# georgeyounes/CRIMP

Measured on AMD Instinct MI355X. Metric: Z^2_2 photon*trial evals/sec (node), higher is better.
Workload: dtype f64; 1 GPU; config3: synthetic 10000000 photons x 1000000 trials/GPU, Z^2_2; photons=10000000, trials_per_gpu=1000000, nharm=2, parallelism=trial-sharded dp1: sharding.sharded_search + all_gather(best), precision=default

## Files before the change

### crimp_amd/csrc/search_nufft.h

```cpp
#pragma once

#include "search_nufft_plan.h"
#include "search_nufft_finish.h"

typedef double nu_f64x4 __attribute__((ext_vector_type(4)));

constexpr int kNuTile = 4096;
constexpr double kNuRho = 1e-13;

struct NuTw {
    const double2* lo;
    const double2* hi;
    int lbits;
    int64_t mask;
};

__device__ __forceinline__ double2 nu_cmul(double2 a, double2 b) {
    return make_double2(a.x * b.x - a.y * b.y, a.x * b.y + a.y * b.x);
}
__device__ __forceinline__ double2 nu_add(double2 a, double2 b) { return make_double2(a.x + b.x, a.y + b.y); }
__device__ __forceinline__ double2 nu_sub(double2 a, double2 b) { return make_double2(a.x - b.x, a.y - b.y); }
__device__ __forceinline__ double2 nu_muli(double2 a) { return make_double2(-a.y, a.x); }

__device__ __forceinline__ double2 nu_tw(const NuTw& T, int64_t t) {
// ... 730 lines not shown
        }
    }
    __syncthreads();
}

__device__ __forceinline__ void nu_fft_lds(double2* s, int ll, int lc, int sa, int sc, const NuTile* tw, int lt) {
    int lns = 0;
    while (lns < ll) {
        const int rem = ll - lns;
        if (rem >= 4) {
            nu_stage<16>(s, ll, lc, sa, sc, lns, tw, lt);
            lns += 4;
        } else if (rem == 3) {
            nu_stage<8>(s, ll, lc, sa, sc, lns, tw, lt);
            lns += 3;
        } else if (rem == 2) {
            nu_stage<4>(s, ll, lc, sa, sc, lns, tw, lt);
            lns += 2;
        } else {
            nu_stage<2>(s, ll, lc, sa, sc, lns, tw, lt);
            lns += 1;
        }
    }
}

__global__ __launch_bounds__(256) __attribute__((amdgpu_waves_per_eu(2))) void k_nu_fft_cols(const double2* __restrict__ X, double2* __restrict__ Y,
                                                     int lnfft, int ln1, int lc, NuTw T, int alo, int acnt) {
    extern __shared__ double2 nu_s[];
    __shared__ NuTile tw;
    const int lt = lnfft < 12 ? lnfft : 12;
    nu_tile_init(&tw, lt);
    const int ln2 = lnfft - ln1, c = 1 << lc, n1 = 1 << ln1;
    const int64_t nfft = int64_t(1) << lnfft;
    const int64_t b0 = (int64_t)blockIdx.x << lc;
    const double2* x = X + (int64_t)blockIdx.y * nfft;
    double2* y = Y + (int64_t)blockIdx.y * nfft;
    for (int e = threadIdx.x; e < (n1 << lc); e += 256) {
        const int a = e >> lc, cc = e & (c - 1);
        nu_s[e] = ((a - alo) & (n1 - 1)) < acnt ? x[((int64_t)a << ln2) + b0 + cc] : make_double2(0.0, 0.0);
    }
    __syncthreads();
    nu_fft_lds(nu_s, ln1, lc, c, 1, &tw, lt);
#pragma unroll
    for (int q = 0; q < kNuTile / 256; ++q) {
        const int e = threadIdx.x + 256 * q;
        if (e < (n1 << lc)) {
            const int k1 = e >> lc, cc = e & (c - 1);
            const int64_t b = b0 + cc;
            y[((int64_t)k1 << ln2) + b] = nu_cmul(nu_s[e], nu_tw(T, b * k1));
        }
    }
}

__global__ __launch_bounds__(256) __attribute__((amdgpu_waves_per_eu(2))) void k_nu_cols256(
    const double2* __restrict__ X, double2* __restrict__ Y, int lnfft, NuTw T, int alo, int acnt, int64_t ngroups) {
    extern __shared__ double2 nu_s[];
    __shared__ NuTile tw;
    nu_tile_init(&tw, 12);
    const int ln2 = lnfft - 8;
    const int64_t nfft = int64_t(1) << lnfft;
    const int cc = threadIdx.x & 15, j = threadIdx.x >> 4;
    const int64_t cpb = int64_t(1) << (ln2 - 4);
    double2 nv[16], tf[4];
    auto fetch = [&](int64_t grp) {
        const int64_t b = ((grp % cpb) << 4) + cc;
        const double2* x = X + (grp / cpb) * nfft + b;
        const int64_t lm = (int64_t(1) << T.lbits) - 1, tb = (b * (int64_t)j) & T.mask, ts = (b << 4) & T.mask;
        tf[0] = T.hi[tb >> T.lbits];
        tf[1] = T.lo[tb & lm];
        tf[2] = T.hi[ts >> T.lbits];
        tf[3] = T.lo[ts & lm];
#pragma unroll
        for (int r = 0; r < 16; ++r) {
            const int a = j + 16 * r;
            nv[r] = ((a - alo) & 255) < acnt ? x[(int64_t)a << ln2] : make_double2(0.0, 0.0);
        }
    };
    int64_t grp = blockIdx.x;
    if (grp < ngroups) fetch(grp);
    __syncthreads();
    for (; grp < ngroups; grp += gridDim.x) {
        double2 v[16];
#pragma unroll
        for (int r = 0; r < 16; ++r) v[r] = nv[r];
        const double2 wb = nu_cmul(tf[0], tf[1]), ws = nu_cmul(tf[2], tf[3]);
        const int64_t b = ((grp % cpb) << 4) + cc;
        double2* y = Y + (grp / cpb) * nfft + b;
        if (grp + gridDim.x < ngroups) fetch(grp + gridDim.x);
        nu_dft16(v);
#pragma unroll
        for (int r = 0; r < 16; ++r) nu_s[((j << 4) + r) * 16 + cc] = v[r];
        __syncthreads();
#pragma unroll
        for (int r = 0; r < 16; ++r) v[r] = nu_s[(j + 16 * r) * 16 + cc];
        __syncthreads();
        nu_twiddle<16>(nu_tw_tile(&tw, j << 4), v);
        nu_dft16(v);
        v[0] = nu_cmul(v[0], wb);
        nu_twiddle<16>(ws, v);
#pragma unroll
        for (int r = 1; r < 16; ++r) v[r] = nu_cmul(v[r], wb);
#pragma unroll
        for (int r = 0; r < 16; ++r) y[(int64_t)(j + 16 * r) << ln2] = v[r];
    }
}

__global__ __launch_bounds__(512) __attribute__((amdgpu_waves_per_eu(4))) void k_nu_cols512(
    const double2* __restrict__ X, double2* __restrict__ Y, int lnfft, NuTw T, int alo, int acnt, int64_t ngroups) {
    constexpr int NC = 1, C = 8;
    extern __shared__ double2 nu_s[];
    __shared__ NuTile tw;
    nu_tile_init(&tw, 9);
    const int ln2 = lnfft - 9;
    const int64_t nfft = int64_t(1) << lnfft;
    const int cc = threadIdx.x & 7, j = threadIdx.x >> 3;
    const int64_t cpb = int64_t(1) << (ln2 - 3);
    double2 nv[NC][8], tf[NC][4];
    const int voff = ((j << ln2) + cc) * 16;
    auto fetch = [&](int64_t grp) {
        const int64_t b0 = (grp % cpb) * C;
        const __amdgpu_buffer_rsrc_t rs = __builtin_amdgcn_make_buffer_rsrc(
            (void*)(X + (grp / cpb) * nfft + b0), (short)0, (int)(16 << lnfft), 0x00020000);
        const int64_t lm = (int64_t(1) << T.lbits) - 1;
#pragma unroll
        for (int c = 0; c < NC; ++c) {
            const int64_t b = b0 + cc + 8 * c, tb = (b * (int64_t)j) & T.mask, ts = (b << 6) & T.mask;
            tf[c][0] = T.hi[tb >> T.lbits];
            tf[c][1] = T.lo[tb & lm];
            tf[c][2] = T.hi[ts >> T.lbits];
            tf[c][3] = T.lo[ts & lm];
        }
#pragma unroll
        for (int q = 0; q < 8; ++q) {
            const bool occ = ((j + 64 * q - alo) & 511) < acnt;
#pragma unroll
            for (int c = 0; c < NC; ++c)
                nv[c][q] = occ ? __builtin_bit_cast(double2, __builtin_amdgcn_raw_buffer_load_b128(
                                                                 rs, voff, ((64 * q << ln2) + 8 * c) * 16, 0))
                               : make_double2(0.0, 0.0);
        }
    };
    int64_t grp = blockIdx.x;
    if (grp < ngroups) fetch(grp);
    const int m2 = (j & 7) << 3;
    const int z2 = ((j >> 3) << 6) + (j & 7);
    __syncthreads();
    typedef unsigned int nu_u4 __attribute__((ext_vector_type(4)));
    for (; grp < ngroups; grp += gridDim.x) {
        double2 v[NC][8], wb[NC], ws[NC];
#pragma unroll
        for (int c = 0; c < NC; ++c) {
#pragma unroll
            for (int q = 0; q < 8; ++q) v[c][q] = nv[c][q];
            wb[c] = nu_cmul(tf[c][0], tf[c][1]);
            ws[c] = nu_cmul(tf[c][2], tf[c][3]);
        }
// ... 78 lines not shown
    }
    for (int p = P - 1; p >= 0; --p) {
        const int64_t pn = (int64_t)(p > 0 ? p - 1 : 0) * pstride;
#pragma unroll
        for (int q = 0; q < kNuFusedPer; ++q) {
            const int e = threadIdx.x + 256 * q;
            if (e < L) {
                nu_s[e] = nx[q];
                nx[q] = xr[pn + e];
            }
        }
        __syncthreads();
        nu_fft_lds(nu_s, ll, 0, 1, L, &tw, lt);
#pragma unroll
        for (int q = 0; q < kNuFusedPer; ++q) {
            const int b = threadIdx.x + 256 * q;
            if (b < L) {
                const double2 v = nu_s[b];
                const int64_t J = k1 + ((int64_t)b << ln1);
                const int64_t jc = J <= jhi ? J : J - nfft;
                acc[q] = nu_bes_acc(acc[q], nu_bes_w(bs[q], p, nu_zh(jc, lnfft)), v, p);
            }
        }
        __syncthreads();
    }
#pragma unroll
    for (int q = 0; q < kNuFusedPer; ++q) {
        const int b = threadIdx.x + 256 * q;
        if (b >= L) continue;
        const int64_t J = k1 + ((int64_t)b << ln1);
        int64_t jc;
        if (J <= jhi)
            jc = J;
        else if (J >= nfft - h)
            jc = J - nfft;
        else
            continue;
        const int64_t t = tbase + r * nf + jc;
        if (t >= 0 && t < nbt) CS[t] = acc[q];
    }
}

struct NuFinal {
    int on, m, stat, Pc;
    double nph, invfact, rel;
    int64_t tb0;
    double* out;
    int* nflag;
    int64_t* flagged;
    BestCand* best_part;
    int64_t best_base;
    const double2* CS0;
};
template <int TPB, int NP>
__device__ __forceinline__ void nu_rows_epilogue(const double2 (&acc)[NP], int64_t k1, int ln1, int64_t nfft,
                                                 int64_t jhi, int64_t h, int64_t tbase, int r, int64_t nf, int64_t nbt,
                                                 double2* __restrict__ CS, const NuFinal& F, double2* lds,
                                                 int pos0 = -1) {
    const int t = threadIdx.x;
    const int b0 = pos0 < 0 ? t : pos0;
    if (!F.on) {
#pragma unroll
        for (int q = 0; q < NP; ++q) {
            const int64_t J = k1 + ((int64_t)(b0 + TPB * q) << ln1);
            int64_t jc;
            if (J <= jhi)
                jc = J;
            else if (J >= nfft - h)
                jc = J - nfft;
            else
                continue;
            const int64_t tt = tbase + r * nf + jc;
            if (tt >= 0 && tt < nbt) CS[tt] = acc[q];
        }
        return;
    }
    BestCand bc_ = {-INFINITY, INT64_MAX};
#pragma unroll
    for (int q = 0; q < NP; ++q) {
        const int64_t J = k1 + ((int64_t)(b0 + TPB * q) << ln1);
        int64_t jc;
        if (J <= jhi)
            jc = J;
        else if (J >= nfft - h)
            jc = J - nfft;
        else
            continue;
        const int64_t tt = tbase + r * nf + jc;
        if (tt < 0 || tt >= nbt) continue;
        double p, err;
        nu_power(F.CS0, nbt, tt, F.m, F.stat, F.nph, nu_err_bound(jc, nfft, F.Pc, F.invfact, F.nph), true, acc[q], &p,
                 &err);
        F.out[F.tb0 + tt] = p;
        if (!(err <= F.rel * fabs(p))) F.flagged[atomicAdd(F.nflag, 1)] = F.tb0 + tt;
        if (best_better(p, F.tb0 + tt, bc_.v, bc_.i)) bc_ = {p, F.tb0 + tt};
    }
    if (!F.best_part) return;
    for (int o = 32; o > 0; o >>= 1) {
        const double v = __shfl_xor(bc_.v, o);
        const int64_t i = __shfl_xor(bc_.i, o);
        if (best_better(v, i, bc_.v, bc_.i)) bc_ = {v, i};
    }
    __syncthreads();
    BestCand* red = reinterpret_cast<BestCand*>(lds);
    if ((t & 63) == 0) red[t >> 6] = bc_;
    __syncthreads();
    if (t == 0) {
        for (int w = 1; w < TPB / 64; ++w)
            if (best_better(red[w].v, red[w].i, bc_.v, bc_.i)) bc_ = red[w];
        F.best_part[F.best_base + (int64_t)blockIdx.y * gridDim.x + blockIdx.x] = bc_;
    }
}

struct NuRot {
// ... 61 lines not shown
        for (int q = 0; q < 8; ++q) v[q] = A[rd + TPB * 9 / 8 * q];
        nu_twiddle<8>(nu_tw_tile(&tw, m2), v);
        nu_dft8(v);
#pragma unroll
        for (int q = 0; q < 8; ++q) B[w2 + Ns2 * q + (q >> 1)] = v[q];
        __syncthreads();
#pragma unroll
        for (int q = 0; q < 8; ++q) v[q] = B[rd + TPB * 9 / 8 * q];
        nu_twiddle<8>(nu_tw_tile(&tw, m3), v);
        nu_dft8(v);
#pragma unroll
        for (int q = 0; q < 8; ++q) A[w3 + Ns3 * 9 / 8 * q] = v[q];
        __syncthreads();
#pragma unroll
        for (int q = 0; q < 8; ++q) v[q] = A[rd + TPB * 9 / 8 * q];
        nu_twiddle<8>(nu_tw_tile(&tw, m4), v);
        nu_dft8(v);
        const double pp1 = (double)(p + 1);
#pragma unroll
        for (int q = 0; q < 8; ++q) {
            const double j = fma(pp1 * bs[q].iz2, bs[q].j1, -bs[q].j2);
            bs[q].j2 = bs[q].j1;
            bs[q].j1 = j;
            double w = j;
            if constexpr (last) w = (q == 0 && k1 == 0 && t == 0) ? 1.0 : 0.5 * j;
            acc[q] = make_double2(fma(w, v[q].x, -acc[q].y), fma(w, v[q].y, acc[q].x));
        }
    };
    const int pend = plo > 0 ? plo : 1;
    int p = P - 1;
    double2* TA = nu_s;
    double2* TB = nu_s + NT;
    if (p >= pend && ((p - pend + 1) & 1)) {
        moment(std::false_type(), p, xa, xb, TA, TB);
        --p;
#pragma unroll
        for (int q = 0; q < 8; ++q) xa[q] = xb[q];
        double2* tt = TA;
        TA = TB;
        TB = tt;
    }
    for (; p >= pend; p -= 2) {
        moment(std::false_type(), p, xa, xb, TA, TB);
        moment(std::false_type(), p - 1, xb, xa, TB, TA);
    }
    if (plo == 0) moment(std::true_type(), 0, xa, xb, TA, TB);
    const int rl = plo & 3;
#pragma unroll
    for (int q = 0; q < 8; ++q) {
        const double2 a = acc[q];
        acc[q] = rl == 0 ? a : rl == 1 ? make_double2(-a.y, a.x) : rl == 2 ? make_double2(-a.x, -a.y)
                                                                : make_double2(a.y, -a.x);
    }
    nu_rows_epilogue<TPB, 8>(acc, k1, ln1, nfft, jhi, h, tbase, r, nf, nbt, CS, F, nu_s);
}

__global__ __launch_bounds__(512) __attribute__((amdgpu_waves_per_eu(2))) void k_nu_rows_iw(
    const double2* X, int lnfft, int P, int plo, int accum, int nrow, int64_t nf, int64_t jhi, int64_t h,
    int64_t tbase, int64_t nbt, const double* __restrict__ bc, double2* __restrict__ CS, const NuFinal F, int xcd) {
    constexpr int N = 4096, TPB = 512;
    extern __shared__ double2 nu_s[];
    __shared__ NuTile tw;
    nu_tile_init(&tw, 12);
    const int64_t nfft = int64_t(1) << lnfft;
    const int ln1 = lnfft - 12;
    const int64_t k1b = nu_row_of_block(blockIdx.x, 1u << ln1, xcd);
    const int r = blockIdx.y;
    const int t = threadIdx.x, w = t >> 6, L = t & 63, hi3 = L >> 3, lo3 = L & 7;
    const int pos0 = w + 8 * hi3 + 64 * lo3;
    const double2* xr = X + (int64_t)r * nfft + (k1b << 12);
    const int64_t pstride = (int64_t)nrow * nfft;
    auto load_row = [&](int pm, double2 (&dst)[8]) {
        const __amdgpu_buffer_rsrc_t rs =
            __builtin_amdgcn_make_buffer_rsrc((void*)(xr + (int64_t)pm * pstride), (short)0, N * 16, 0x00020000);
#pragma unroll
        for (int q = 0; q < 8; ++q)
            dst[q] = __builtin_bit_cast(double2, __builtin_amdgcn_raw_buffer_load_b128(rs, t * 16, TPB * 16 * q, 0));
    };
    double2 acc[8], xa[8], xb[8];
    NuRot bs[8];
    const int rP = P & 3;
#pragma unroll
    for (int q = 0; q < 8; ++q) {
        double2 a0 = make_double2(0.0, 0.0);
        const int64_t J = k1b + ((int64_t)(pos0 + TPB * q) << ln1);
        const int64_t jc = J <= jhi ? J : J - nfft;
        if (accum) {
            const int64_t tt = tbase + r * nf + jc;
            if ((J <= jhi || J >= nfft - h) && tt >= 0 && tt < nbt) a0 = CS[tt];
        }
        acc[q] = rP == 0 ? a0 : rP == 1 ? make_double2(a0.y, -a0.x) : rP == 2 ? make_double2(-a0.x, -a0.y)
                                                                        : make_double2(-a0.y, a0.x);
        const NuBes b0 = nu_bes_start(bc, P, nu_zh(jc, lnfft));
        bs[q] = {2.0 * b0.j1, 2.0 * b0.j2, b0.iz2};
    }
    load_row(P - 1 - plo, xa);
    const int cw = 64 * w + L, cr = 512 * w + L, e1w = 512 * w + 64 * hi3 + lo3, e2w = 512 * w + 8 * hi3,
              e2r = 512 * w + 64 * lo3 + 8 * hi3;
    __syncthreads();
    auto moment = [&](auto LAST, int p, double2 (&v)[8], double2 (&nv)[8], double2* A) {
        constexpr bool last = decltype(LAST)::value;
        if (p > plo) load_row(p - 1 - plo, nv);
        nu_dft8(v);
        nu_twiddle<8>(nu_tw_tile(&tw, t), v);
#pragma unroll
        for (int q = 0; q < 8; ++q) A[cw + 512 * q] = v[q];
        __syncthreads();
#pragma unroll
        for (int q = 0; q < 8; ++q) v[q] = A[cr + 64 * q];
        nu_dft8(v);
        nu_twiddle<8>(nu_tw_tile(&tw, 8 * L), v);
#pragma unroll
        for (int q = 0; q < 8; ++q) A[e1w + 8 * q] = v[q];
        asm volatile("s_waitcnt lgkmcnt(0)" ::: "memory");
#pragma unroll
        for (int q = 0; q < 8; ++q) v[q] = A[cr + 64 * q];
        nu_dft8(v);
        nu_twiddle<8>(nu_tw_tile(&tw, 64 * lo3), v);
#pragma unroll
        for (int q = 0; q < 8; ++q) A[e2w + 64 * q + (lo3 ^ q)] = v[q];
        asm volatile("s_waitcnt lgkmcnt(0)" ::: "memory");
#pragma unroll
        for (int q = 0; q < 8; ++q) v[q] = A[e2r + (q ^ lo3)];
        nu_dft8(v);
        const double pp1 = (double)(p + 1);
#pragma unroll
        for (int q = 0; q < 8; ++q) {
            const double j = fma(pp1 * bs[q].iz2, bs[q].j1, -bs[q].j2);
            bs[q].j2 = bs[q].j1;
            bs[q].j1 = j;
            double wgt = j;
            if constexpr (last) wgt = (q == 0 && k1b == 0 && pos0 == 0) ? 1.0 : 0.5 * j;
            acc[q] = make_double2(fma(wgt, v[q].x, -acc[q].y), fma(wgt, v[q].y, acc[q].x));
        }
    };
    const int pend = plo > 0 ? plo : 1;
    int p = P - 1;
    double2* TA = nu_s;
    double2* TB = nu_s + N;
    if (p >= pend && ((p - pend + 1) & 1)) {
        moment(std::false_type(), p, xa, xb, TA);
        --p;
#pragma unroll
        for (int q = 0; q < 8; ++q) xa[q] = xb[q];
        double2* tt = TA;
        TA = TB;
        TB = tt;
    }
    for (; p >= pend; p -= 2) {
        moment(std::false_type(), p, xa, xb, TA);
        moment(std::false_type(), p - 1, xb, xa, TB);
    }
    if (plo == 0) moment(std::true_type(), 0, xa, xb, TA);
    const int rl = plo & 3;
#pragma unroll
    for (int q = 0; q < 8; ++q) {
        const double2 a = acc[q];
        acc[q] = rl == 0 ? a : rl == 1 ? make_double2(-a.y, a.x) : rl == 2 ? make_double2(-a.x, -a.y)
                                                                : make_double2(a.y, -a.x);
    }
    nu_rows_epilogue<TPB, 8>(acc, k1b, ln1, nfft, jhi, h, tbase, r, nf, nbt, CS, F, nu_s, pos0);
}

__global__ __launch_bounds__(256) void k_nu_finalize(const double2* __restrict__ CS, int64_t nbt, int m, int stat,
                                                     double nph, int64_t nf, int64_t jbase, int64_t nfft, int P,
                                                     double invfact, double rel, int64_t tb0, int64_t first,
                                                     double* __restrict__ out, int* __restrict__ nflag,
                                                     int64_t* __restrict__ flagged) {
    const int64_t t = (int64_t)blockIdx.x * blockDim.x + threadIdx.x;
    if (t >= nbt) return;
    const int64_t flat = tb0 + t + first;
    const int64_t jc = flat % nf - jbase;
    double p, err;
    nu_power(CS, nbt, t, m, stat, nph, nu_err_bound(jc, nfft, P, invfact, nph), false, make_double2(0.0, 0.0), &p,
             &err);
    out[tb0 + t] = p;
    if (!(err <= rel * fabs(p))) flagged[atomicAdd(nflag, 1)] = tb0 + t;
}

static int g_last_search_path = 0;
static int64_t g_last_nufft_n = 0;
static int g_last_nufft_p = 0;
static int g_last_nufft_gather = 0;
static double g_nu_work[kNuCls] = {0, 0, 0, 0, 0, 0, 0};
static int64_t g_last_cells_built = 0, g_last_cells_reused = 0;

struct NuTables {
    NuTw T{};
    const double2* cis = nullptr;
    const double2* cis2 = nullptr;
    const double* bc = nullptr;
};
static int nu_tables(hipStream_t s, int lnfft, NuTables* out) {
    static std::mutex mu;
    static std::map<std::pair<int, int>, double2*> cache;
    const int lbits = std::min(lnfft, 11);
    const int64_t nlo = int64_t(1) << lbits, nhi = int64_t(1) << (lnfft - lbits);
    int dev = 0;
    HIPCHK(hipGetDevice(&dev));
    double2* d = nullptr;
    {
        std::lock_guard<std::mutex> lk(mu);
        auto it = cache.find({dev, lnfft});
        if (it != cache.end()) {
            d = it->second;
        } else {
            std::vector<double2> h((size_t)(nlo + nhi + 1024 + kNuBesP * kNuBesM / 2 + 2048));
            const long double tp = 6.283185307179586476925286766559L;
            const long double nf = (long double)(int64_t(1) << lnfft);
            for (int64_t i = 0; i < nlo; ++i) {
                const long double a = tp * (long double)i / nf;
                h[(size_t)i] = make_double2((double)cosl(a), (double)sinl(a));
            }
            for (int64_t i = 0; i < nhi; ++i) {
// ... 311 lines not shown
        else if (sp.starts_max > 0)
            HIPCHK(sc.alloc(&cstart, (size_t)sp.starts_max));
        HIPCHK(sc.alloc(&W, (size_t)(sp.Bmax * sp.gw)));
        HIPCHK(sc.alloc(&Y, (size_t)sp.Bmax));
        HIPCHK(sc.alloc(&CS, (size_t)sp.csmax));
        HIPCHK(sc.alloc(&flagged, (size_t)in.shape.count));
        if (best_host)
            best_part = reinterpret_cast<BestCand*>(reinterpret_cast<char*>(in.nflag) + kNuFinCandOff);
        else if (sp.best_alloc > 0)
            HIPCHK(sc.alloc(&best_part, (size_t)sp.best_alloc));
        if (!sp.passes.empty()) {
            HIPCHK(sc.alloc(&dps, sp.passes.size()));
            HIPCHK(hipMemcpyAsync(dps, sp.passes.data(), sp.passes.size() * sizeof(NuPass), hipMemcpyHostToDevice, s));
        }
        return CRIMP_OK;
    }

    int cell_starts(const NuGroup& g, int64_t base) {
        const int64_t n = in.shape.n;
        for (const NuCellLaunch& cl : g.cells) {
            NuCellArgs ca = cl.args;
            for (int j = 0; j < cl.nk; ++j) ca.off[j] += base;
            const unsigned cb = (unsigned)std::min<int64_t>(cdiv(cdiv(n, 2), 256 * kNuCellU), 2048);
            if ((reinterpret_cast<uintptr_t>(in.t) & 15u) == 0)
                k_nu_cellstart<true><<<cb, 256, 0, s>>>(in.t, in.t0, n, g.pl.s1, cl.k0, cl.nk, ca, cstart, in.nflag + 1);
            else
                k_nu_cellstart<false><<<cb, 256, 0, s>>>(in.t, in.t0, n, g.pl.s1, cl.k0, cl.nk, ca, cstart, in.nflag + 1);
            HIPCHK(hipGetLastError());
        }
        HIPCHK(span(kNuClsCellStart));
        return CRIMP_OK;
    }

    int gather_set(const NuGroup& g, const NuBatch& b, const NuGatherSet& set, int64_t base) {
        const NuPlan& pl = g.pl;
        NuGatherSet S = set;
        for (int jj = 0; jj < S.nk; ++jj) S.soff[jj] += base;
        NuFold F;
        if (fold) {
            char* blkp = reinterpret_cast<char*>(in.nflag);
            F.epoch = epoch;
            F.ncheck = first_gather ? ncheck : 0;
            F.f = in.freq;
            F.nf = in.shape.nf;
            F.n = in.shape.n;
            F.pub = reinterpret_cast<double*>(blkp + kNuFinPubOff);
            F.part = reinterpret_cast<double2*>(blkp + kNuFinPartOff);
        }
        first_gather = false;
        launch_gather(in.twod, cells_reuse, S.blk0[S.nk], in.t, in.t0, cstart, int64_t(1) << pl.lnfft, pl.s1, pl.fch,
                      pl.fcl, in.twod ? in.c2 + b.rb : nullptr, b.nrow, pl.P, S, in.nflag + 1, tab.cis2, W, F, s);
        HIPCHK(hipGetLastError());
        HIPCHK(span(kNuClsSpread));
        for (int jj = 0; jj < S.nk; ++jj) {
            const int rc = fft_combine(g, b, S.k[jj], W + S.woff[jj]);
            if (rc) return rc;
        }
        return CRIMP_OK;
    }

    int mfma_pass(const NuGroup& g, const NuBatch& b, const NuMfmaPass& mp) {
        const NuPlan& pl = g.pl;
        const int64_t n = in.shape.n, nchunk = sp.nchunk, nfft = int64_t(1) << pl.lnfft;
        const int64_t SL = 2 * (int64_t)pl.P * b.nrow;
        const NuPass& ps = sp.passes[mp.ipass];
        const NuPass* dp = dps + mp.ipass;
        const dim3 grid((unsigned)cdiv(nchunk, kNuWaves));
        if (in.twod)
            nu_launch_spread<true>(mp.gl, grid, s, in.t, in.t0, n, nchunk, pl.s1, pl.fch, pl.fcl, in.c2 + b.rb, b.nrow,
                                   mp.k0, pl.P, dp, tab.cis, U, ctab, in.nflag + 1);
        else
            nu_launch_spread<false>(mp.gl, grid, s, in.t, in.t0, n, nchunk, pl.s1, pl.fch, pl.fcl, in.c2 + b.rb, b.nrow,
                                    mp.k0, pl.P, dp, tab.cis, U, ctab, in.nflag + 1);
        HIPCHK(hipGetLastError());
        HIPCHK(span(kNuClsSpread));
        for (int kk = 0; kk < mp.gl && mp.k0 + kk <= in.shape.nharm; ++kk) {
            const int k = mp.k0 + kk;
            int alo = 0, acnt = 0;
            nu_occupied(pl.gmin[(size_t)(k - 1)], pl.gmax[(size_t)(k - 1)], pl.lnfft, g.ln1, &alo, &acnt);
            const int64_t gbase = (int64_t)alo << g.ln2, gcount = (int64_t)acnt << g.ln2;
            k_nu_merge<<<(unsigned)cdiv(gcount, kNuMergeG), 256, (size_t)kNuMergeG * SL * sizeof(double), s>>>(
                U + ps.ubase[kk], SL, ctab + 2 * kk * nchunk, nchunk, ps.gmin[kk], pl.gmax[(size_t)(k - 1)], nfft, gbase,
                gcount, W, in.nflag + 1);
            HIPCHK(hipGetLastError());
            HIPCHK(span(kNuClsMerge));
            const int rc = fft_combine(g, b, k, W);
            if (rc) return rc;
        }
        return CRIMP_OK;
    }

    int fft_combine(const NuGroup& g, const NuBatch& b, int k, const double2* Wk) {
        const NuPlan& pl = g.pl;
        const NuSearchShape& sh = in.shape;
        const bool generic_fft = in.hooks.generic_fft;
        const int lnfft = pl.lnfft, P = pl.P, ln1 = g.ln1, ln2 = g.ln2;
        const size_t lds_fft = (size_t)kNuTile * sizeof(double2);
        const int64_t Bp = (int64_t)P * b.nrow;
        const double2* Z = Wk;
        if (ln1 > 0) {
            const int lcol = 12 - ln1;
            int alo = 0, acnt = 0;
            nu_occupied(pl.gmin[(size_t)(k - 1)], pl.gmax[(size_t)(k - 1)], lnfft, ln1, &alo, &acnt);
            if (ln1 == 8 && !generic_fft) {
                const int64_t ngroups = Bp << (ln2 - 4);
                k_nu_cols256<<<(unsigned)std::min<int64_t>(ngroups, 2 * nu_cus()), 256, lds_fft, s>>>(
                    Wk, Y, lnfft, tab.T, alo, acnt, ngroups);
            } else if (ln1 == 9 && !generic_fft) {
                const int64_t ngroups = Bp << (ln2 - 3);
                k_nu_cols512<<<(unsigned)std::min<int64_t>(ngroups, 2 * nu_cus()), 512, lds_fft, s>>>(
                    Wk, Y, lnfft, tab.T, alo, acnt, ngroups);
            } else {
                k_nu_fft_cols<<<dim3((unsigned)(int64_t(1) << (ln2 - lcol)), (unsigned)Bp), 256, lds_fft, s>>>(
                    Wk, Y, lnfft, ln1, lcol, tab.T, alo, acnt);
            }
            HIPCHK(hipGetLastError());
            Z = Y;
            HIPCHK(span(kNuClsPass1));
        }
        NuFinal F{};
        if (g.fuse_final && k == sh.nharm) {
            F.on = 1;
            F.m = sh.nharm;
            F.stat = sh.stat;
            F.Pc = P;
            F.nph = (double)sh.n;
            F.invfact = pl.invfact;
            F.rel = in.search_hooks.fixup_rel;
            F.tb0 = b.tb0;
            F.out = in.out;
            F.nflag = in.nflag;
            F.flagged = flagged;
            F.best_part = in.best ? best_part : nullptr;
            F.best_base = b.best_base;
            F.CS0 = CS;
        }
        const dim3 g2((unsigned)(int64_t(1) << ln1), (unsigned)b.nrow);
        const int xcd = in.hooks.row_map;
        const int64_t jhi = pl.nseg - 1 - pl.h, tbase = b.rb * sh.nf + g.jbase - (b.tb0 + sh.first);
        double2* CSk = CS + (int64_t)(k - 1) * b.nbt;
        if (ln2 == 12 && !generic_fft)
            k_nu_rows_iw<<<g2, 512, 2 * lds_fft, s>>>(Z, lnfft, P, 0, 0, b.nrow, sh.nf, jhi, pl.h, tbase, b.nbt, tab.bc,
                                                      CSk, F, xcd);
        else if (ln2 == 11 && !generic_fft)
            k_nu_rows_combine8<11><<<g2, 256, nu_rows_lds(11), s>>>(Z, lnfft, P, 0, 0, b.nrow, sh.nf, jhi, pl.h, tbase,
                                                                     b.nbt, tab.bc, CSk, F);
        else
            k_nu_fft_rows_combine<<<g2, 256, lds_fft, s>>>(Z, ln2, lnfft, P, b.nrow, sh.nf, jhi, pl.h, tbase, b.nbt,
                                                           tab.bc, CSk, xcd);
        HIPCHK(hipGetLastError());
        HIPCHK(span(kNuClsPass2));
        return CRIMP_OK;
    }

    int finalize(const NuGroup& g, const NuBatch& b) {
        const NuSearchShape& sh = in.shape;
        k_nu_finalize<<<(unsigned)cdiv(b.nbt, 256), 256, 0, s>>>(CS, b.nbt, sh.nharm, sh.stat, (double)sh.n, sh.nf, g.jbase,
                                                                 int64_t(1) << g.pl.lnfft, g.pl.P, g.pl.invfact,
                                                                 in.search_hooks.fixup_rel, b.tb0, sh.first, in.out, in.nflag, flagged);
        HIPCHK(hipGetLastError());
        HIPCHK(span(kNuClsFinalize));
        return CRIMP_OK;
    }

    int launch_all() {
        int cur_lnfft = -1;
        for (const NuGroup& g : sp.groups) {
            int rc = CRIMP_OK;
            if (g.pl.lnfft != cur_lnfft) {
                rc = nu_tables(s, g.pl.lnfft, &tab);
                if (rc) return rc;
                cur_lnfft = g.pl.lnfft;
            }
            if (ev.empty()) HIPCHK(mark());
            const int64_t base = cells_reuse || cells_keep ? g.starts_off : 0;
            if (sp.gather && !cells_reuse) {
                rc = cell_starts(g, base);
                if (rc) return rc;
            }
            for (const NuBatch& b : g.batches) {
                for (const NuGatherSet& S : b.sets) {
                    rc = gather_set(g, b, S, base);
                    if (rc) return rc;
                }
                for (const NuMfmaPass& mp : b.mfma) {
                    rc = mfma_pass(g, b, mp);
                    if (rc) return rc;
                }
                if (g.fuse_final) continue;
                rc = finalize(g, b);
                if (rc) return rc;
            }
        }
        return CRIMP_OK;
    }

    int report_times() {
        if (!in.timed) return CRIMP_OK;
        HIPCHK(hipEventSynchronize(ev.back()));
        float tot = 0.0f;
        double cls[kNuCls] = {0, 0, 0, 0, 0, 0, 0};
        HIPCHK(hipEventElapsedTime(&tot, ev.front(), ev.back()));
// ... 116 lines not shown
```

### crimp_amd/csrc/search_nufft_plan.h

```cpp
#pragma once

#include <algorithm>
#include <cmath>
#include <cstdint>
#include <cstdlib>
#include <cstring>
#include <utility>
#include <vector>

constexpr int kNuCW = 1024;
constexpr int kNuWaves = 4;
constexpr int kNuRows = 8;
constexpr int kNuMaxP = 16;
constexpr int kNuGatherMaxP = 24;
constexpr int kNuMergeG = 16;
constexpr int kNuMaxWrap = 32;
constexpr double kNuEps = 5e-14;
constexpr double kNuEpsZm = 5e-13;

constexpr int kNuPassMax = 10;
struct NuPass {
    int64_t gmin[kNuPassMax];
    int64_t ubase[kNuPassMax];
};
// ... 6 lines not shown
constexpr int kNuGatherRows = 2;
constexpr int kNuGatherSet = 8;
struct NuGatherSet {
    int nk;
    int k[kNuGatherSet], lanes_log2[kNuGatherSet];
    int64_t blk0[kNuGatherSet + 1];
    int64_t gmin[kNuGatherSet], gmax[kNuGatherSet], gbase[kNuGatherSet], gcount[kNuGatherSet];
    int64_t soff[kNuGatherSet], woff[kNuGatherSet];
};

enum { kNuClsCellStart, kNuClsSpread, kNuClsMerge, kNuClsPass1, kNuClsPass2, kNuClsCombine, kNuClsFinalize, kNuCls };

inline int64_t nu_cdiv(int64_t a, int64_t b) { return (a + b - 1) / b; }

inline double nu_trunc(double x, int P, double* invfact) {
    double f = 1.0, xp = 1.0;
    for (int p = 1; p <= P; ++p) {
        f *= 2.0 * (double)p;
        xp *= x;
    }
    *invfact = 2.4 / f;
    return 2.4 * xp / f;
}

inline int ilog2(int64_t v) {
    int l = 0;
    while ((int64_t(1) << l) < v) ++l;
    return l;
}

inline void nu_occupied(int64_t gmin, int64_t gmax, int lnfft, int ln1, int* alo, int* acnt) {
    const int64_t nfft = int64_t(1) << lnfft, n1 = int64_t(1) << ln1;
    const int ln2 = lnfft - ln1;
    *alo = 0;
    *acnt = (int)n1;
    if (ln1 == 0 || gmax - gmin + 1 >= nfft) return;
    const int64_t glo = gmin & (nfft - 1), ghi = glo + (gmax - gmin);
    const int64_t a0 = glo >> ln2, a1 = ghi >> ln2;
    if (a1 - a0 + 1 >= n1) return;
    *alo = (int)a0;
    *acnt = (int)(a1 - a0 + 1);
}

struct NuHooks {
    enum { kAuto, kGather, kMfma };
    int spread = kAuto;
    int lanes = 0;
    bool generic_fft = false;
    bool separate_final = false;
    bool plan_cache_off = false;
    bool cell_cache_off = false;
    bool fold_off = false;
    int row_map = 1;
    int64_t budget = int64_t(6144) << 20;
    int64_t cell_cap = int64_t(64) << 20;

    bool lanes_valid() const { return lanes == 0 || lanes == 1 || lanes == 2 || lanes == 4 || lanes == 8; }
    void set_budget(int64_t bytes) {
        budget = bytes;
        cell_cap = std::min<int64_t>(bytes / 32, int64_t(64) << 20);
    }
    static NuHooks from_env() {
        static const int64_t budget_env = [] {
            const char* e = getenv("CRIMP_NUFFT_BUDGET_MB");
            const long long mb = e ? atoll(e) : 6144;
            return (int64_t)(mb > 0 ? mb : 6144) << 20;
        }();
        auto is = [](const char* name, const char* val) {
            const char* e = getenv(name);
            return e && !strcmp(e, val);
        };
        NuHooks h;
        h.spread = is("CRIMP_NUFFT_SPREAD", "gather") ? kGather : is("CRIMP_NUFFT_SPREAD", "mfma") ? kMfma : kAuto;
        const char* lanes_s = getenv("CRIMP_NUFFT_LANES");
        h.lanes = lanes_s ? atoi(lanes_s) : 0;
        h.generic_fft = is("CRIMP_NUFFT_ROWS4096", "0");
        h.separate_final = is("CRIMP_NUFFT_FINAL", "separate");
        h.plan_cache_off = is("CRIMP_NUFFT_PLAN_CACHE", "0");
        h.cell_cache_off = is("CRIMP_NUFFT_CELL_CACHE", "0");
        h.fold_off = is("CRIMP_NUFFT_FOLD", "0");
        h.row_map = is("CRIMP_NUFFT_ROW_MAP", "linear") ? 0 : 1;
        h.set_budget(budget_env);
        return h;
    }
};

struct NuPlan {
    int64_t r0 = 0, r1 = 0, j0 = 0, nseg = 0, h = 0;
    int lnfft = 0, P = 0;
    double invfact = 1.0, s1 = 0.0, fch = 0.0, fcl = 0.0;
    std::vector<int64_t> gmin, gmax;
};

inline bool nu_plan(NuPlan* pl, double delta, double f0, double dt0, double dtn, int nharm, int pmax, double eps) {
    if (!(delta > 0.0) || !std::isfinite(delta) || !std::isfinite(f0)) return false;
    const int64_t h = pl->nseg / 2;
    pl->h = h;
    int lnfft = 0, P = 0;
    double invfact = 1.0;
    for (int l = std::max(ilog2(pl->nseg), 6); l <= 24; ++l) {
        const double x = M_PI * (double)std::max<int64_t>(h, pl->nseg - 1 - h) / (double)(int64_t(1) << l);
        int p = 1;
        while (p <= pmax && nu_trunc(x, p, &invfact) > eps) ++p;
        if (p > pmax) continue;
        if (lnfft == 0 || ((int64_t)p << l) < ((int64_t)P << lnfft)) {
            lnfft = l;
            P = p;
        }
        if (p <= 4) break;
    }
    if (lnfft == 0) return false;
    nu_trunc(0.0, P, &invfact);
    pl->lnfft = lnfft;
    pl->P = P;
    pl->invfact = invfact;
    const int64_t nfft = int64_t(1) << lnfft;
    pl->s1 = (double)nfft * delta;
    const double c = (double)(pl->j0 + h);
    const double hp = c * delta, hpe = std::fma(c, delta, -hp);
    const double fch = f0 + hp, bb = fch - f0;
    pl->fch = fch;
    pl->fcl = ((f0 - (fch - bb)) + (hp - bb)) + hpe;
    const double u0 = dt0 * pl->s1, un = dtn * pl->s1;
    const double glim = 2147483647.0 - (double)nfft;
    pl->gmin.assign((size_t)nharm, 0);
    pl->gmax.assign((size_t)nharm, 0);
    for (int k = 1; k <= nharm; ++k) {
        const double a = (double)k * u0, b = (double)k * un;
        if (!(std::fabs(a) < glim && std::fabs(b) < glim)) return false;
        pl->gmin[(size_t)(k - 1)] = (int64_t)std::rint(a);
        pl->gmax[(size_t)(k - 1)] = (int64_t)std::rint(b);
        if (pl->gmax[(size_t)(k - 1)] < pl->gmin[(size_t)(k - 1)]) return false;
        if ((pl->gmax[(size_t)(k - 1)] - pl->gmin[(size_t)(k - 1)]) / nfft + 1 > kNuMaxWrap) return false;
    }
// ... 312 lines not shown
```

Measured before the change: 29090000 billion equivalent photon*trial evals/s.

## Batch harmonic set into single column and row FFT kernel launches

When several harmonics share a spread group, the column FFT (cols256) and the row/combine kernel (rows_iw) now process all harmonics of the set in one launch. Previously each harmonic got its own pair of launches. Column passes run in place on W with buffer-resource loads and stores, and the row kernel loops over harmonics, fusing the final statistic only on the last one. The aim is to cut launch count and tail inefficiency on small grids, at the cost of more register and scalar pressure and new env-controlled paths.

```diff
diff --git a/crimp_amd/csrc/search_nufft.h b/crimp_amd/csrc/search_nufft.h
--- a/crimp_amd/csrc/search_nufft.h
+++ b/crimp_amd/csrc/search_nufft.h
@@ -806,19 +806,37 @@
     }
 }
 
+struct NuColsSet {
+    int nk;
+    int alo[kNuGatherSet], acnt[kNuGatherSet];
+    int64_t woff[kNuGatherSet];
+};
 __global__ __launch_bounds__(256) __attribute__((amdgpu_waves_per_eu(2))) void k_nu_cols256(
-    const double2* __restrict__ X, double2* __restrict__ Y, int lnfft, NuTw T, int alo, int acnt, int64_t ngroups) {
+    const double2* X, double2* Y, int lnfft, NuTw T, const NuColsSet C, int64_t gph, int64_t ngroups) {
     extern __shared__ double2 nu_s[];
     __shared__ NuTile tw;
     nu_tile_init(&tw, 12);
     const int ln2 = lnfft - 8;
-    const int64_t nfft = int64_t(1) << lnfft;
     const int cc = threadIdx.x & 15, j = threadIdx.x >> 4;
     const int64_t cpb = int64_t(1) << (ln2 - 4);
     double2 nv[16], tf[4];
+    const int voff = ((j << ln2) + cc) * 16;
+    auto locate = [&](int64_t grp, int* hh, int64_t* b0) {
+        int h = 0;
+#pragma unroll
+        for (int i = 1; i < kNuGatherSet; ++i) h += grp >= i * gph ? 1 : 0;
+        const int64_t gl = grp - h * gph;
+        *hh = h;
+        *b0 = (gl & (cpb - 1)) << 4;
+        return C.woff[h] + ((gl >> (ln2 - 4)) << lnfft) + *b0;
+    };
     auto fetch = [&](int64_t grp) {
-        const int64_t b = ((grp % cpb) << 4) + cc;
-        const double2* x = X + (grp / cpb) * nfft + b;
+        int hh;
+        int64_t b0;
+        const __amdgpu_buffer_rsrc_t rs = __builtin_amdgcn_make_buffer_rsrc(
+            (void*)(X + locate(grp, &hh, &b0)), (short)0, (int)(16 << lnfft), 0x00020000);
+        const int alo = C.alo[hh], acnt = C.acnt[hh];
+        const int64_t b = b0 + cc;
         const int64_t lm = (int64_t(1) << T.lbits) - 1, tb = (b * (int64_t)j) & T.mask, ts = (b << 4) & T.mask;
         tf[0] = T.hi[tb >> T.lbits];
         tf[1] = T.lo[tb & lm];
@@ -827,19 +845,24 @@
 #pragma unroll
         for (int r = 0; r < 16; ++r) {
             const int a = j + 16 * r;
-            nv[r] = ((a - alo) & 255) < acnt ? x[(int64_t)a << ln2] : make_double2(0.0, 0.0);
+            nv[r] = ((a - alo) & 255) < acnt
+                        ? __builtin_bit_cast(double2, __builtin_amdgcn_raw_buffer_load_b128(rs, voff, (16 * r << ln2) * 16, 0))
+                        : make_double2(0.0, 0.0);
         }
     };
     int64_t grp = blockIdx.x;
     if (grp < ngroups) fetch(grp);
     __syncthreads();
+    typedef unsigned int nu_u4 __attribute__((ext_vector_type(4)));
     for (; grp < ngroups; grp += gridDim.x) {
         double2 v[16];
 #pragma unroll
         for (int r = 0; r < 16; ++r) v[r] = nv[r];
         const double2 wb = nu_cmul(tf[0], tf[1]), ws = nu_cmul(tf[2], tf[3]);
-        const int64_t b = ((grp % cpb) << 4) + cc;
-        double2* y = Y + (grp / cpb) * nfft + b;
+        int hh;
+        int64_t b0;
+        const __amdgpu_buffer_rsrc_t ry = __builtin_amdgcn_make_buffer_rsrc(
+            (void*)(Y + locate(grp, &hh, &b0)), (short)0, (int)(16 << lnfft), 0x00020000);
         if (grp + gridDim.x < ngroups) fetch(grp + gridDim.x);
         nu_dft16(v);
 #pragma unroll
@@ -855,7 +878,8 @@
 #pragma unroll
         for (int r = 1; r < 16; ++r) v[r] = nu_cmul(v[r], wb);
 #pragma unroll
-        for (int r = 0; r < 16; ++r) y[(int64_t)(j + 16 * r) << ln2] = v[r];
+        for (int r = 0; r < 16; ++r)
+            __builtin_amdgcn_raw_buffer_store_b128(__builtin_bit_cast(nu_u4, v[r]), ry, voff, (16 * r << ln2) * 16, 0);
     }
 }
 
@@ -1040,14 +1064,18 @@
     int64_t best_base;
     const double2* CS0;
 };
+struct NuRowsSet {
+    int nk;
+    int64_t xoff[kNuGatherSet], csoff[kNuGatherSet];
+};
 template <int TPB, int NP>
 __device__ __forceinline__ void nu_rows_epilogue(const double2 (&acc)[NP], int64_t k1, int ln1, int64_t nfft,
                                                  int64_t jhi, int64_t h, int64_t tbase, int r, int64_t nf, int64_t nbt,
-                                                 double2* __restrict__ CS, const NuFinal& F, double2* lds,
+                                                 double2* CS, const NuFinal& F, int on, double2* lds,
                                                  int pos0 = -1) {
     const int t = threadIdx.x;
     const int b0 = pos0 < 0 ? t : pos0;
-    if (!F.on) {
+    if (!on) {
 #pragma unroll
         for (int q = 0; q < NP; ++q) {
             const int64_t J = k1 + ((int64_t)(b0 + TPB * q) << ln1);
@@ -1215,114 +1243,125 @@
         acc[q] = rl == 0 ? a : rl == 1 ? make_double2(-a.y, a.x) : rl == 2 ? make_double2(-a.x, -a.y)
                                                                 : make_double2(a.y, -a.x);
     }
-    nu_rows_epilogue<TPB, 8>(acc, k1, ln1, nfft, jhi, h, tbase, r, nf, nbt, CS, F, nu_s);
+    nu_rows_epilogue<TPB, 8>(acc, k1, ln1, nfft, jhi, h, tbase, r, nf, nbt, CS, F, F.on, nu_s);
 }
 
 __global__ __launch_bounds__(512) __attribute__((amdgpu_waves_per_eu(2))) void k_nu_rows_iw(
-    const double2* X, int lnfft, int P, int plo, int accum, int nrow, int64_t nf, int64_t jhi, int64_t h,
-    int64_t tbase, int64_t nbt, const double* __restrict__ bc, double2* __restrict__ CS, const NuFinal F, int xcd) {
+    const double2* X, int lnfft_a, int P_a, int plo, int accum, int nrow, int64_t nf, int64_t jhi, int64_t h,
+    int64_t tbase, int64_t nbt, const double* __restrict__ bc, double2* CS, const NuFinal F_a, int xcd,
+    const NuRowsSet R) {
     constexpr int N = 4096, TPB = 512;
     extern __shared__ double2 nu_s[];
     __shared__ NuTile tw;
     nu_tile_init(&tw, 12);
-    const int64_t nfft = int64_t(1) << lnfft;
-    const int ln1 = lnfft - 12;
-    const int64_t k1b = nu_row_of_block(blockIdx.x, 1u << ln1, xcd);
     const int r = blockIdx.y;
-    const int t = threadIdx.x, w = t >> 6, L = t & 63, hi3 = L >> 3, lo3 = L & 7;
-    const int pos0 = w + 8 * hi3 + 64 * lo3;
-    const double2* xr = X + (int64_t)r * nfft + (k1b << 12);
-    const int64_t pstride = (int64_t)nrow * nfft;
-    auto load_row = [&](int pm, double2 (&dst)[8]) {
-        const __amdgpu_buffer_rsrc_t rs =
-            __builtin_amdgcn_make_buffer_rsrc((void*)(xr + (int64_t)pm * pstride), (short)0, N * 16, 0x00020000);
-#pragma unroll
-        for (int q = 0; q < 8; ++q)
-            dst[q] = __builtin_bit_cast(double2, __builtin_amdgcn_raw_buffer_load_b128(rs, t * 16, TPB * 16 * q, 0));
-    };
-    double2 acc[8], xa[8], xb[8];
-    NuRot bs[8];
-    const int rP = P & 3;
-#pragma unroll
-    for (int q = 0; q < 8; ++q) {
-        double2 a0 = make_double2(0.0, 0.0);
-        const int64_t J = k1b + ((int64_t)(pos0 + TPB * q) << ln1);
-        const int64_t jc = J <= jhi ? J : J - nfft;
-        if (accum) {
-            const int64_t tt = tbase + r * nf + jc;
-            if ((J <= jhi || J >= nfft - h) && tt >= 0 && tt < nbt) a0 = CS[tt];
-        }
-        acc[q] = rP == 0 ? a0 : rP == 1 ? make_double2(a0.y, -a0.x) : rP == 2 ? make_double2(-a0.x, -a0.y)
-                                                                        : make_double2(-a0.y, a0.x);
-        const NuBes b0 = nu_bes_start(bc, P, nu_zh(jc, lnfft));
-        bs[q] = {2.0 * b0.j1, 2.0 * b0.j2, b0.iz2};
-    }
-    load_row(P - 1 - plo, xa);
-    const int cw = 64 * w + L, cr = 512 * w + L, e1w = 512 * w + 64 * hi3 + lo3, e2w = 512 * w + 8 * hi3,
-              e2r = 512 * w + 64 * lo3 + 8 * hi3;
-    __syncthreads();
-    auto moment = [&](auto LAST, int p, double2 (&v)[8], double2 (&nv)[8], double2* A) {
-        constexpr bool last = decltype(LAST)::value;
-        if (p > plo) load_row(p - 1 - plo, nv);
-        nu_dft8(v);
-        nu_twiddle<8>(nu_tw_tile(&tw, t), v);
-#pragma unroll
-        for (int q = 0; q < 8; ++q) A[cw + 512 * q] = v[q];
+#pragma unroll 1
+    for (int ih = 0; ih < R.nk; ++ih) {
+        int t = threadIdx.x, lnfft = lnfft_a, P = P_a;
+        NuFinal F = F_a;
+        asm volatile("" : "+v"(t));
+        asm volatile("" : "+s"(bc), "+s"(lnfft), "+s"(P));
+        asm volatile("" : "+s"(F.nph), "+s"(F.invfact), "+s"(F.rel), "+s"(F.Pc), "+s"(F.m), "+s"(F.stat));
+        const int64_t nfft = int64_t(1) << lnfft;
+        const int ln1 = lnfft - 12;
+        const int64_t k1b = nu_row_of_block(blockIdx.x, 1u << ln1, xcd);
+        const int w = t >> 6, L = t & 63, hi3 = L >> 3, lo3 = L & 7;
+        const int pos0 = w + 8 * hi3 + 64 * lo3;
+        double2* CSh = CS + R.csoff[ih];
+        const int fin = F.on && ih == R.nk - 1;
+        const double2* xr = X + R.xoff[ih] + (int64_t)r * nfft + (k1b << 12);
+        const int64_t pstride = (int64_t)nrow * nfft;
+        auto load_row = [&](int pm, double2 (&dst)[8]) {
+            const __amdgpu_buffer_rsrc_t rs =
+                __builtin_amdgcn_make_buffer_rsrc((void*)(xr + (int64_t)pm * pstride), (short)0, N * 16, 0x00020000);
+#pragma unroll
+            for (int q = 0; q < 8; ++q)
+                dst[q] = __builtin_bit_cast(double2, __builtin_amdgcn_raw_buffer_load_b128(rs, t * 16, TPB * 16 * q, 0));
+        };
+        double2 acc[8], xa[8], xb[8];
+        NuRot bs[8];
+        const int rP = P & 3;
+#pragma unroll
+        for (int q = 0; q < 8; ++q) {
+            double2 a0 = make_double2(0.0, 0.0);
+            const int64_t J = k1b + ((int64_t)(pos0 + TPB * q) << ln1);
+            const int64_t jc = J <= jhi ? J : J - nfft;
+            if (accum) {
+                const int64_t tt = tbase + r * nf + jc;
+                if ((J <= jhi || J >= nfft - h) && tt >= 0 && tt < nbt) a0 = CSh[tt];
+            }
+            acc[q] = rP == 0 ? a0 : rP == 1 ? make_double2(a0.y, -a0.x) : rP == 2 ? make_double2(-a0.x, -a0.y)
+                                                                            : make_double2(-a0.y, a0.x);
+            const NuBes b0 = nu_bes_start(bc, P, nu_zh(jc, lnfft));
+            bs[q] = {2.0 * b0.j1, 2.0 * b0.j2, b0.iz2};
+        }
+        load_row(P - 1 - plo, xa);
+        const int cw = 64 * w + L, cr = 512 * w + L, e1w = 512 * w + 64 * hi3 + lo3, e2w = 512 * w + 8 * hi3,
+                  e2r = 512 * w + 64 * lo3 + 8 * hi3;
         __syncthreads();
-#pragma unroll
-        for (int q = 0; q < 8; ++q) v[q] = A[cr + 64 * q];
-        nu_dft8(v);
-        nu_twiddle<8>(nu_tw_tile(&tw, 8 * L), v);
-#pragma unroll
-        for (int q = 0; q < 8; ++q) A[e1w + 8 * q] = v[q];
-        asm volatile("s_waitcnt lgkmcnt(0)" ::: "memory");
-#pragma unroll
-        for (int q = 0; q < 8; ++q) v[q] = A[cr + 64 * q];
-        nu_dft8(v);
-        nu_twiddle<8>(nu_tw_tile(&tw, 64 * lo3), v);
-#pragma unroll
-        for (int q = 0; q < 8; ++q) A[e2w + 64 * q + (lo3 ^ q)] = v[q];
-        asm volatile("s_waitcnt lgkmcnt(0)" ::: "memory");
-#pragma unroll
-        for (int q = 0; q < 8; ++q) v[q] = A[e2r + (q ^ lo3)];
-        nu_dft8(v);
-        const double pp1 = (double)(p + 1);
+        auto moment = [&](auto LAST, int p, double2 (&v)[8], double2 (&nv)[8], double2* A) {
+            constexpr bool last = decltype(LAST)::value;
+            if (p > plo) load_row(p - 1 - plo, nv);
+            nu_dft8(v);
+            nu_twiddle<8>(nu_tw_tile(&tw, t), v);
+#pragma unroll
+            for (int q = 0; q < 8; ++q) A[cw + 512 * q] = v[q];
+            __syncthreads();
+#pragma unroll
+            for (int q = 0; q < 8; ++q) v[q] = A[cr + 64 * q];
+            nu_dft8(v);
+            nu_twiddle<8>(nu_tw_tile(&tw, 8 * L), v);
+#pragma unroll
+            for (int q = 0; q < 8; ++q) A[e1w + 8 * q] = v[q];
+            asm volatile("s_waitcnt lgkmcnt(0)" ::: "memory");
+#pragma unroll
+            for (int q = 0; q < 8; ++q) v[q] = A[cr + 64 * q];
+            nu_dft8(v);
+            nu_twiddle<8>(nu_tw_tile(&tw, 64 * lo3), v);
+#pragma unroll
+            for (int q = 0; q < 8; ++q) A[e2w + 64 * q + (lo3 ^ q)] = v[q];
+            asm volatile("s_waitcnt lgkmcnt(0)" ::: "memory");
+#pragma unroll
+            for (int q = 0; q < 8; ++q) v[q] = A[e2r + (q ^ lo3)];
+            nu_dft8(v);
+            const double pp1 = (double)(p + 1);
+#pragma unroll
+            for (int q = 0; q < 8; ++q) {
+                const double j = fma(pp1 * bs[q].iz2, bs[q].j1, -bs[q].j2);
+                bs[q].j2 = bs[q].j1;
+                bs[q].j1 = j;
+                double wgt = j;
+                if constexpr (last) wgt = (q == 0 && k1b == 0 && pos0 == 0) ? 1.0 : 0.5 * j;
+                acc[q] = make_double2(fma(wgt, v[q].x, -acc[q].y), fma(wgt, v[q].y, acc[q].x));
+            }
+        };
+        const int pend = plo > 0 ? plo : 1;
+        int p = P - 1;
+        double2* TA = nu_s;
+        double2* TB = nu_s + N;
+        if (p >= pend && ((p - pend + 1) & 1)) {
+            moment(std::false_type(), p, xa, xb, TA);
+            --p;
+#pragma unroll
+            for (int q = 0; q < 8; ++q) xa[q] = xb[q];
+            double2* tt = TA;
+            TA = TB;
+            TB = tt;
+        }
+        for (; p >= pend; p -= 2) {
+            moment(std::false_type(), p, xa, xb, TA);
+            moment(std::false_type(), p - 1, xb, xa, TB);
+        }
+        if (plo == 0) moment(std::true_type(), 0, xa, xb, TA);
+        const int rl = plo & 3;
 #pragma unroll
         for (int q = 0; q < 8; ++q) {
-            const double j = fma(pp1 * bs[q].iz2, bs[q].j1, -bs[q].j2);
-            bs[q].j2 = bs[q].j1;
-            bs[q].j1 = j;
-            double wgt = j;
-            if constexpr (last) wgt = (q == 0 && k1b == 0 && pos0 == 0) ? 1.0 : 0.5 * j;
-            acc[q] = make_double2(fma(wgt, v[q].x, -acc[q].y), fma(wgt, v[q].y, acc[q].x));
-        }
-    };
-    const int pend = plo > 0 ? plo : 1;
-    int p = P - 1;
-    double2* TA = nu_s;
-    double2* TB = nu_s + N;
-    if (p >= pend && ((p - pend + 1) & 1)) {
-        moment(std::false_type(), p, xa, xb, TA);
-        --p;
-#pragma unroll
-        for (int q = 0; q < 8; ++q) xa[q] = xb[q];
-        double2* tt = TA;
-        TA = TB;
-        TB = tt;
-    }
-    for (; p >= pend; p -= 2) {
-        moment(std::false_type(), p, xa, xb, TA);
-        moment(std::false_type(), p - 1, xb, xa, TB);
-    }
-    if (plo == 0) moment(std::true_type(), 0, xa, xb, TA);
-    const int rl = plo & 3;
-#pragma unroll
-    for (int q = 0; q < 8; ++q) {
-        const double2 a = acc[q];
-        acc[q] = rl == 0 ? a : rl == 1 ? make_double2(-a.y, a.x) : rl == 2 ? make_double2(-a.x, -a.y)
-                                                                : make_double2(a.y, -a.x);
-    }
-    nu_rows_epilogue<TPB, 8>(acc, k1b, ln1, nfft, jhi, h, tbase, r, nf, nbt, CS, F, nu_s, pos0);
+            const double2 a = acc[q];
+            acc[q] = rl == 0 ? a : rl == 1 ? make_double2(-a.y, a.x) : rl == 2 ? make_double2(-a.x, -a.y)
+                                                                    : make_double2(a.y, -a.x);
+        }
+        nu_rows_epilogue<TPB, 8>(acc, k1b, ln1, nfft, jhi, h, tbase, r, nf, nbt, CSh, F, fin, nu_s, pos0);
+    }
 }
 
 __global__ __launch_bounds__(256) void k_nu_finalize(const double2* __restrict__ CS, int64_t nbt, int m, int stat,
@@ -1740,11 +1779,51 @@
                       pl.fcl, in.twod ? in.c2 + b.rb : nullptr, b.nrow, pl.P, S, in.nflag + 1, tab.cis2, W, F, s);
         HIPCHK(hipGetLastError());
         HIPCHK(span(kNuClsSpread));
+        const bool spec = !in.hooks.generic_fft, inplace = spec && g.ln1 == 8;
+        const bool set_cols = S.nk > 1 && inplace && (in.hooks.harm_set & NuHooks::kCols);
+        const bool set_rows = S.nk > 1 && spec && g.ln2 == 12 && (g.ln1 == 0 || inplace) &&
+                              (in.hooks.harm_set & NuHooks::kRows);
+        if (!set_cols && !set_rows) {
+            for (int jj = 0; jj < S.nk; ++jj) {
+                const int rc = fft_combine(g, b, S.k[jj], W + S.woff[jj]);
+                if (rc) return rc;
+            }
+            return CRIMP_OK;
+        }
+        if (g.ln1 > 0) {
+            NuColsSet C{};
+            for (int jj = 0; jj < S.nk; ++jj) {
+                nu_occupied(pl.gmin[(size_t)(S.k[jj] - 1)], pl.gmax[(size_t)(S.k[jj] - 1)], pl.lnfft, g.ln1,
+                            &C.alo[jj], &C.acnt[jj]);
+                C.woff[jj] = S.woff[jj];
+            }
+            if (set_cols) {
+                C.nk = S.nk;
+                HIPCHK(cols256(g, b, W, W, C));
+            } else {
+                for (int jj = 0; jj < S.nk; ++jj) {
+                    NuColsSet C1{};
+                    C1.nk = 1;
+                    C1.alo[0] = C.alo[jj];
+                    C1.acnt[0] = C.acnt[jj];
+                    HIPCHK(cols256(g, b, W + S.woff[jj], W + S.woff[jj], C1));
+                }
+            }
+        }
+        if (set_rows) return fft_rows(g, b, S.k, S.woff, S.nk, W);
         for (int jj = 0; jj < S.nk; ++jj) {
-            const int rc = fft_combine(g, b, S.k[jj], W + S.woff[jj]);
+            const int rc = fft_rows(g, b, S.k + jj, S.woff + jj, 1, W);
             if (rc) return rc;
         }
         return CRIMP_OK;
+    }
+
+    hipError_t cols256(const NuGroup& g, const NuBatch& b, const double2* X, double2* Yo, const NuColsSet& C) {
+        const int64_t gph = ((int64_t)g.pl.P * b.nrow) << (g.ln2 - 4), ngroups = gph * C.nk;
+        k_nu_cols256<<<(unsigned)std::min<int64_t>(ngroups, 2 * nu_cus()), 256, (size_t)kNuTile * sizeof(double2), s>>>(
+            X, Yo, g.pl.lnfft, tab.T, C, gph, ngroups);
+        const hipError_t e = hipGetLastError();
+        return e != hipSuccess ? e : span(kNuClsPass1);
     }
 
     int mfma_pass(const NuGroup& g, const NuBatch& b, const NuMfmaPass& mp) {
@@ -1780,7 +1859,6 @@
 
     int fft_combine(const NuGroup& g, const NuBatch& b, int k, const double2* Wk) {
         const NuPlan& pl = g.pl;
-        const NuSearchShape& sh = in.shape;
         const bool generic_fft = in.hooks.generic_fft;
         const int lnfft = pl.lnfft, P = pl.P, ln1 = g.ln1, ln2 = g.ln2;
         const size_t lds_fft = (size_t)kNuTile * sizeof(double2);
@@ -1791,9 +1869,13 @@
             int alo = 0, acnt = 0;
             nu_occupied(pl.gmin[(size_t)(k - 1)], pl.gmax[(size_t)(k - 1)], lnfft, ln1, &alo, &acnt);
             if (ln1 == 8 && !generic_fft) {
-                const int64_t ngroups = Bp << (ln2 - 4);
-                k_nu_cols256<<<(unsigned)std::min<int64_t>(ngroups, 2 * nu_cus()), 256, lds_fft, s>>>(
-                    Wk, Y, lnfft, tab.T, alo, acnt, ngroups);
+                NuColsSet C{};
+                C.nk = 1;
+                C.alo[0] = alo;
+                C.acnt[0] = acnt;
+                HIPCHK(cols256(g, b, Wk, Y, C));
+                const int64_t zero = 0;
+                return fft_rows(g, b, &k, &zero, 1, Y);
             } else if (ln1 == 9 && !generic_fft) {
                 const int64_t ngroups = Bp << (ln2 - 3);
                 k_nu_cols512<<<(unsigned)std::min<int64_t>(ngroups, 2 * nu_cus()), 512, lds_fft, s>>>(
@@ -1806,8 +1888,18 @@
             Z = Y;
             HIPCHK(span(kNuClsPass1));
         }
+        const int64_t zero = 0;
+        return fft_rows(g, b, &k, &zero, 1, Z);
+    }
+
+    int fft_rows(const NuGroup& g, const NuBatch& b, const int* ks, const int64_t* xoff, int nk, const double2* Z) {
+        const NuPlan& pl = g.pl;
+        const NuSearchShape& sh = in.shape;
+        const bool generic_fft = in.hooks.generic_fft;
+        const int lnfft = pl.lnfft, P = pl.P, ln1 = g.ln1, ln2 = g.ln2;
+        const size_t lds_fft = (size_t)kNuTile * sizeof(double2);
         NuFinal F{};
-        if (g.fuse_final && k == sh.nharm) {
+        if (g.fuse_final && ks[nk - 1] == sh.nharm) {
             F.on = 1;
             F.m = sh.nharm;
             F.stat = sh.stat;
@@ -1826,16 +1918,25 @@
         const dim3 g2((unsigned)(int64_t(1) << ln1), (unsigned)b.nrow);
         const int xcd = in.hooks.row_map;
         const int64_t jhi = pl.nseg - 1 - pl.h, tbase = b.rb * sh.nf + g.jbase - (b.tb0 + sh.first);
-        double2* CSk = CS + (int64_t)(k - 1) * b.nbt;
-        if (ln2 == 12 && !generic_fft)
+        double2* CSk = CS + (int64_t)(ks[0] - 1) * b.nbt;
+        if (ln2 == 12 && !generic_fft) {
+            NuRowsSet R{};
+            R.nk = nk;
+            for (int jj = 0; jj < nk; ++jj) {
+                R.xoff[jj] = xoff[jj];
+                R.csoff[jj] = (int64_t)(ks[jj] - 1) * b.nbt;
+            }
             k_nu_rows_iw<<<g2, 512, 2 * lds_fft, s>>>(Z, lnfft, P, 0, 0, b.nrow, sh.nf, jhi, pl.h, tbase, b.nbt, tab.bc,
-                                                      CSk, F, xcd);
-        else if (ln2 == 11 && !generic_fft)
-            k_nu_rows_combine8<11><<<g2, 256, nu_rows_lds(11), s>>>(Z, lnfft, P, 0, 0, b.nrow, sh.nf, jhi, pl.h, tbase,
-                                                                     b.nbt, tab.bc, CSk, F);
-        else
-            k_nu_fft_rows_combine<<<g2, 256, lds_fft, s>>>(Z, ln2, lnfft, P, b.nrow, sh.nf, jhi, pl.h, tbase, b.nbt,
-                                                           tab.bc, CSk, xcd);
+                                                      CS, F, xcd, R);
+        } else if (nk != 1) {
+            return set_err(CRIMP_ERR_ARG, "nufft: a set of harmonics needs the 4096-element row kernel");
+        } else if (ln2 == 11 && !generic_fft) {
+            k_nu_rows_combine8<11><<<g2, 256, nu_rows_lds(11), s>>>(Z + xoff[0], lnfft, P, 0, 0, b.nrow, sh.nf, jhi, pl.h,
+                                                                     tbase, b.nbt, tab.bc, CSk, F);
+        } else {
+            k_nu_fft_rows_combine<<<g2, 256, lds_fft, s>>>(Z + xoff[0], ln2, lnfft, P, b.nrow, sh.nf, jhi, pl.h, tbase,
+                                                           b.nbt, tab.bc, CSk, xcd);
+        }
         HIPCHK(hipGetLastError());
         HIPCHK(span(kNuClsPass2));
         return CRIMP_OK;
diff --git a/crimp_amd/csrc/search_nufft_plan.h b/crimp_amd/csrc/search_nufft_plan.h
--- a/crimp_amd/csrc/search_nufft_plan.h
+++ b/crimp_amd/csrc/search_nufft_plan.h
@@ -82,6 +82,8 @@
     bool cell_cache_off = false;
     bool fold_off = false;
     int row_map = 1;
+    enum { kCols = 1, kRows = 2 };
+    int harm_set = kCols | kRows;
     int64_t budget = int64_t(6144) << 20;
     int64_t cell_cap = int64_t(64) << 20;
 
@@ -110,6 +112,10 @@
         h.cell_cache_off = is("CRIMP_NUFFT_CELL_CACHE", "0");
         h.fold_off = is("CRIMP_NUFFT_FOLD", "0");
         h.row_map = is("CRIMP_NUFFT_ROW_MAP", "linear") ? 0 : 1;
+        h.harm_set = is("CRIMP_NUFFT_HARM_SET", "0")      ? 0
+                     : is("CRIMP_NUFFT_HARM_SET", "cols") ? kCols
+                     : is("CRIMP_NUFFT_HARM_SET", "rows") ? kRows
+                                                          : kCols | kRows;
         h.set_budget(budget_env);
         return h;
     }
```

Result: slower. 28140000 billion equivalent photon*trial evals/s (-3.3%).
